# aleju/cat-generator

Measured on AMD Instinct MI355X. Metric: images/sec per G+D step, G32up-c 32x32 RGB bs=128 per GPU, higher is better.
Workload: dtype f32

## Files before the change

cat-generator_amd/csrc/common.h:

```cpp
#pragma once
#include <hip/hip_runtime.h>
#include <algorithm>
#include <stdint.h>
#include <stdio.h>
#include <string.h>
#include "../../include/catgan.h"

namespace cg {

char* err_buf();
int fail(const char* fmt, ...);

inline hipStream_t S(void* s) { return reinterpret_cast<hipStream_t>(s); }

#define CG_HIP(call)                                                              \
    do {                                                                          \
        hipError_t e__ = (call);                                                  \
        if (e__ != hipSuccess)                                                    \
            return cg::fail("%s:%d %s -> %s", __FILE__, __LINE__, #call,          \
                            hipGetErrorString(e__));                              \
    } while (0)

#define CG_LAUNCH_CHECK()                                                         \
    do {                                                                          \
        hipError_t e__ = hipGetLastError();                                       \
        if (e__ != hipSuccess)                                                    \
            return cg::fail("%s:%d kernel launch -> %s", __FILE__, __LINE__,      \
                            hipGetErrorString(e__));                              \
    } while (0)

#define CG_REQUIRE(cond, ...)                                                     \
    do {                                                                          \
        if (!(cond)) return cg::fail(__VA_ARGS__);                                \
    } while (0)

constexpr int kNumCU = 256;

#ifndef CG_TIMING_PROBE
#define CG_TIMING_PROBE 0
#endif
#define CG_PROBE_HALF(fam, T) (((CG_TIMING_PROBE) & (fam)) ? ((T) + 1) / 2 : (T))
constexpr int kEwWgsPerCU = 4, kColReduceWgsPerCU = 1;

enum Opt {
    OPT_SKINNY, OPT_GEMM_BK32, OPT_WINO_BK, OPT_NN_TILE, OPT_TN_TILE, OPT_NN_SPLITS, OPT_TN_SPLITS,
    OPT_XCD_SWIZZLE, OPT_NN_GLDS, OPT_TN_GLDS, OPT_WINO_GLDS, OPT_PAD_SKIP, OPT_WINO3, OPT_COUNT
};
long opt(Opt o);

static inline int cdiv(long a, long b) { return (int)((a + b - 1) / b); }

constexpr size_t kColScratchBytes = 8u << 20;
void* col_scratch(hipStream_t stream);
hipStream_t queue_stream(hipStream_t ref, int cls, int slot);
int queue_class(hipStream_t ref, hipStream_t s);
void wgrad_discard_all();

bool skinny_mfma_ok(int Cin, int Cout, int H, int W);
int skinny_mfma_forward(hipStream_t st, const float* x, const float* w, const float* bias, float* y, int N, int H, int W, int Cin, int Cout);
int skinny_mfma_wgrad(hipStream_t st, const float* x, const float* dy, float* part, float* bias_part, int N, int H, int W, int Cin, int Cout,
                      int max_blocks);

bool head_wgrad_ok(int N, int T, int C, int Co);
int head_wgrad(hipStream_t st, const float* x, const float* dy, float* gw, float* gb, int N, int T, int C, int Co, float scale);
bool wino3_geom_ok(int ngroups, int N, int H, int W, int Cin, int Cout, int kH, int kW, int padH, int padW, int ups);
int wino3_note_pack(hipStream_t st, int n, const float* const* w, float* const* wf, float* const* wb, const int* Cout, const int* Cin,
                    const int* kH, const int* kW, const int* wb_map);
int wino3_forward(hipStream_t st, int ngroups, const float* const* x, const float* const* wpk, const float* const* bias, float* const* y,
                  int N, int H, int W);

static inline int ew_grid(long n, int per_block = 256) {
    long b = (n + per_block - 1) / per_block;
    if (b < 1) b = 1;
    const long cap = (long)kNumCU * kEwWgsPerCU;
    if (b > cap) b = cap;
    return (int)b;
}

__device__ __forceinline__ float u01(uint64_t seed, uint64_t ctr) {
    uint64_t z = seed + (ctr + 1) * 0x9E3779B97F4A7C15ull;
    z = (z ^ (z >> 30)) * 0xBF58476D1CE4E5B9ull;
    z = (z ^ (z >> 27)) * 0x94D049BB133111EBull;
    z = z ^ (z >> 31);
    return (float)(z >> 40) * (1.0f / 16777216.0f);
}
__device__ __forceinline__ float wave_sum(float v) {
#pragma unroll
    for (int off = 32; off > 0; off >>= 1) v += __shfl_down(v, off, 64);
    return v;
// ... 112 lines not shown
```

cat-generator_amd/csrc/gemm.hip:

```cpp
#include "common.h"
#include <stdlib.h>
#include <algorithm>
#include <mutex>
#include <type_traits>
#include <unordered_map>
#include <vector>

namespace {

typedef float f32x16 __attribute__((ext_vector_type(16)));
typedef unsigned int u32x4 __attribute__((ext_vector_type(4)));

constexpr int BK = 16;
constexpr unsigned OOB = 0x80000000u;
#ifdef CG_TRACE
__device__ unsigned long long* g_trace;
#define CG_STAMP(slot)                                                                                                  \
    do {                                                                                                                \
        if (threadIdx.x == 0 && g_trace) {                                                                              \
            const long wg = blockIdx.x + (long)gridDim.x * (blockIdx.y + (long)gridDim.y * blockIdx.z);                  \
            g_trace[wg * 8 + (slot)] = wall_clock64();                                                                  \
            if ((slot) == 0) {                                                                                          \
                g_trace[wg * 8 + 4] = __builtin_amdgcn_s_getreg((31 << 11) | 4);                       \
                g_trace[wg * 8 + 5] = __builtin_amdgcn_s_getreg((31 << 11) | 20);                     \
// ... 1320 lines not shown
#pragma unroll
            for (int r = 0; r < 16; ++r) {
                const int soff = (i * 32 + (r & 3) + 8 * (r >> 2)) * c4;
#pragma unroll
                for (int j = 0; j < NI; ++j)
                    __builtin_amdgcn_raw_buffer_store_b32(__float_as_uint(acc[i][j][r]), rp, (int)(vo + j * 128), soff, 0);
            }
        return;
    }
#pragma unroll
    for (int j = 0; j < NI; ++j) {
        const int n = n0 + wn0 + j * 32 + l31;
        if (n >= g.Cout) continue;
#pragma unroll
        for (int i = 0; i < MI; ++i) {
#pragma unroll
            for (int r = 0; r < 16; ++r) {
                const int m = m0 + wm0 + i * 32 + (r & 3) + 8 * (r >> 2) + 4 * h;
                if (m < g.Ktot) pout[(long)m * g.Cout + n] = acc[i][j][r];
            }
        }
    }
}

__device__ __host__ __forceinline__ int phase_map(int a, int d, int pad) { return ((a + d - pad) >> 1) - ((a - pad) >> 1); }

template <bool UPS>
__global__ __launch_bounds__(256) void wgrad_reduce_kernel(const float* part, float* gw, int Cin, int Cout, int k, int KK,
                                                           int pad, int kp, int S, float scale, int CI_T, long sstride) {
    extern __shared__ float sh[];
    const int ci0 = blockIdx.x * CI_T, co0 = blockIdx.y * 32;
    const long plane = (long)(UPS ? kp * kp : KK) * Cin * Cout;
    const int n1 = KK * CI_T * 32;
    if (UPS && k == 3 && kp == 2 && pad == 1 && co0 + 32 <= Cout && ci0 + CI_T <= Cin && (CI_T & 31) == 0 && (Cout & 3) == 0 && ((uintptr_t)part & 15) == 0 &&
        (sstride & 3) == 0) {
        const int c4 = threadIdx.x & 7;
        for (int ci_l = threadIdx.x >> 3; ci_l < CI_T; ci_l += 32) {
            float4 acc[9];
#pragma unroll
            for (int t = 0; t < 9; ++t) acc[t] = make_float4(0.f, 0.f, 0.f, 0.f);
            const float* base = part + (long)(ci0 + ci_l) * Cout + co0 + 4 * c4;
            for (int sp = 0; sp < S; ++sp) {
                float4 v[4][4];
#pragma unroll
                for (int p = 0; p < 4; ++p)
#pragma unroll
                    for (int tp = 0; tp < 4; ++tp) v[p][tp] = ld4(base + (long)sp * sstride + (long)p * plane + (long)tp * Cin * Cout);
#pragma unroll
                for (int t = 0; t < 9; ++t) {
                    const int dy = t / 3, dx = t - 3 * (t / 3);
#pragma unroll
                    for (int p = 0; p < 4; ++p) {
                        const float4 q = v[p][phase_map(p >> 1, dy, 1) * 2 + phase_map(p & 1, dx, 1)];
                        acc[t].x += q.x; acc[t].y += q.y; acc[t].z += q.z; acc[t].w += q.w;
                    }
                }
            }
#pragma unroll
            for (int t = 0; t < 9; ++t) {
                float* d = sh + (ci_l * KK + t) * 33 + 4 * c4;
                d[0] = acc[t].x; d[1] = acc[t].y; d[2] = acc[t].z; d[3] = acc[t].w;
            }
        }
    } else
    for (int idx = threadIdx.x; idx < n1; idx += 256) {
        const int co_l = idx & 31;
        const int r = idx >> 5;
        const int ci_l = r % CI_T, tap = r / CI_T;
        const int ci = ci0 + ci_l, co = co0 + co_l;
        float s = 0.f;
        if (ci < Cin && co < Cout) {
            if (UPS) {
                const int dy = tap / k, dx = tap - dy * k;
                for (int sp = 0; sp < S; ++sp)
#pragma unroll
                    for (int p = 0; p < 4; ++p) {
                        const int tp = phase_map(p >> 1, dy, pad) * kp + phase_map(p & 1, dx, pad);
                        s += part[(long)sp * sstride + (long)p * plane + ((long)tp * Cin + ci) * Cout + co];
                    }
            } else {
                const long o = ((long)tap * Cin + ci) * Cout + co;
                for (int sp = 0; sp < S; ++sp) s += part[(long)sp * sstride + o];
            }
        }
        sh[(ci_l * KK + tap) * 33 + co_l] = s;
    }
    __syncthreads();
    const int run = CI_T * KK;
    for (int idx = threadIdx.x; idx < n1; idx += 256) {
        const int j = idx % run, co_l = idx / run;
        const int ci_l = j / KK, tap = j - ci_l * KK;
        const int ci = ci0 + ci_l, co = co0 + co_l;
        if (ci < Cin && co < Cout) {
            float* dst = gw + ((long)co * Cin + ci) * KK + tap;
            *dst += scale * sh[j * 33 + co_l];
        }
    }
}

struct RedPtrs { float* gw0; float* gw1; float* gw2; float* gw3; float* gb0; float* gb1; float* gb2; float* gb3;
                 long gws; };

template <bool UPS>
__device__ __forceinline__ void wgrad_reduce_small_body(float (*sh)[33], int bx, int group, const float* part, const float* bias_part,
                                                        const RedPtrs& rp, int Cin, int Cout, int k, int KK, int pad, int kp, int S,
                                                        int P, float scale, long sstride, long gstride, long bsstride, int wblocks) {
    const int ol = threadIdx.x & 31, ln = threadIdx.x >> 5;
    float s = 0.f;
    if (bx < wblocks) {
        const long total = (long)KK * Cin * Cout;
        const long plane = (long)(UPS ? kp * kp : KK) * Cin * Cout;
        const long i = bx * 32L + ol;
        const float* pg = part + (long)group * gstride;
        int co = 0, ci = 0, tap = 0;
        if (i < total) {
            co = (int)(i % Cout);
            const long r = i / Cout;
            ci = (int)(r % Cin);
            tap = (int)(r / Cin);
            if (UPS) {
                const int dy = tap / k, dx = tap - dy * k;
                for (int sp = ln; sp < S; sp += 8)
#pragma unroll
                    for (int p = 0; p < 4; ++p) {
                        const int tp = phase_map(p >> 1, dy, pad) * kp + phase_map(p & 1, dx, pad);
                        s += pg[(long)sp * sstride + (long)p * plane + ((long)tp * Cin + ci) * Cout + co];
                    }
            } else {
#pragma unroll 4
// ... 970 lines not shown
size_t cg_conv2d_wgrad_workspace_bytes(int N, int Hp, int Wp, int Cin, int Cout, int kH, int kW, int padH, int padW,
                                       int ups) {
    return cg_conv2d_wgrad_workspace_bytes_grouped(1, N, Hp, Wp, Cin, Cout, kH, kW, padH, padW, ups);
}

namespace {
std::mutex g_red_mu;
std::unordered_map<hipStream_t, std::vector<RedJob>> g_red_queue;

long red_cap() { return 0x7fffffffL; }

int small_reduce(hipStream_t st, bool defer, const RedJob& job, int ngroups) {
    if (defer) {
        std::lock_guard<std::mutex> lk(g_red_mu);
        g_red_queue[st].push_back(job);
        g_red_queue[st].back().block0 = ngroups;
        return 0;
    }
    const int nblocks = job.wblocks + job.bblocks;
    const long cap = std::max<long>(1, red_cap() / std::max(1, ngroups));
    dim3 sgrid((unsigned)std::min<long>(nblocks, cap), ngroups);
    if (job.ups)
        hipLaunchKernelGGL(wgrad_reduce_small_kernel<true>, sgrid, dim3(256), 0, st, job.part, job.bias_part, job.rp, job.Cin, job.Cout,
                           job.k, job.KK, job.pad, job.kp, job.S, job.P, job.scale, job.sstride, job.gstride, job.bsstride, job.wblocks, nblocks, 0);
    else
        hipLaunchKernelGGL(wgrad_reduce_small_kernel<false>, sgrid, dim3(256), 0, st, job.part, job.bias_part, job.rp, job.Cin, job.Cout,
                           job.k, job.KK, job.pad, job.kp, job.S, job.P, job.scale, job.sstride, job.gstride, job.bsstride, job.wblocks, nblocks, job.v4);
    CG_LAUNCH_CHECK();
    return 0;
}

int wgrad_impl(void* stream, int ngroups, const float* const* x, const float* const* dy, float* const* gw, float* const* gb, int N,
               int Hp, int Wp, int Cin, int Cout, int kH, int kW, int padH, int padW, int ups, float scale, void* ws, size_t ws_bytes,
               bool defer, long xgs = 0, long dgs = 0, long gws = 0, bool gemm_only = false);
}

int cg_conv2d_wgrad_grouped(void* stream, int ngroups, const float* const* x, const float* const* dy, float* const* gw,
                            float* const* gb, int N, int Hp, int Wp, int Cin, int Cout, int kH, int kW, int padH, int padW,
                            int ups, float scale, void* ws, size_t ws_bytes) {
    return wgrad_impl(stream, ngroups, x, dy, gw, gb, N, Hp, Wp, Cin, Cout, kH, kW, padH, padW, ups, scale, ws, ws_bytes, false);
}

int cg_conv2d_wgrad_grouped_deferred(void* stream, int ngroups, const float* const* x, const float* const* dy, float* const* gw,
                                     float* const* gb, int N, int Hp, int Wp, int Cin, int Cout, int kH, int kW, int padH, int padW,
                                     int ups, float scale, void* ws, size_t ws_bytes) {
    return wgrad_impl(stream, ngroups, x, dy, gw, gb, N, Hp, Wp, Cin, Cout, kH, kW, padH, padW, ups, scale, ws, ws_bytes, true);
}

int cg_conv2d_wgrad_strided(void* stream, int ngroups, const float* x, long x_stride, const float* dy, long dy_stride, float* gw,
                            long gw_stride, int N, int Hp, int Wp, int Cin, int Cout, int kH, int kW, int padH, int padW, int ups,
                            float scale, void* ws, size_t ws_bytes) {
    CG_REQUIRE(x && dy && gw && x_stride > 0 && dy_stride > 0 && gw_stride > 0, "cg_conv2d_wgrad_strided: bad arguments");
    CG_REQUIRE(ngroups >= 1 && ngroups <= kMaxStridedGroups, "cg_conv2d_wgrad_strided: 1..%d groups per launch", kMaxStridedGroups);
    return wgrad_impl(stream, ngroups, &x, &dy, &gw, nullptr, N, Hp, Wp, Cin, Cout, kH, kW, padH, padW, ups, scale, ws, ws_bytes, false,
                      x_stride, dy_stride, gw_stride);
}

int cg_conv2d_wgrad_gemm(void* stream, const float* x, const float* dy, int N, int Hp, int Wp, int Cin, int Cout, int kH, int kW, int padH,
                         int padW, int ups, void* ws, size_t ws_bytes) {
    CG_REQUIRE(x && dy && ws, "cg_conv2d_wgrad_gemm: null pointer");
    CG_REQUIRE(!skinny_ok(1, Cin, Cout, kH, kW, padH, padW, ups), "cg_conv2d_wgrad_gemm: this geometry runs the skinny kernel, not the GEMM");
    float* gw = (float*)ws;
    return wgrad_impl(stream, 1, &x, &dy, &gw, nullptr, N, Hp, Wp, Cin, Cout, kH, kW, padH, padW, ups, 1.f, ws, ws_bytes, false, 0, 0, 0, true);
}

int cg_conv2d_wgrad_pending(void* stream, int* njobs) {
    CG_REQUIRE(njobs, "cg_conv2d_wgrad_pending: null pointer");
    std::lock_guard<std::mutex> lk(g_red_mu);
    auto it = g_red_queue.find(cg::S(stream));
    *njobs = it == g_red_queue.end() ? 0 : (int)it->second.size();
    return 0;
}

int cg_conv2d_wgrad_flush(void* stream) {
    hipStream_t st = cg::S(stream);
    std::vector<RedJob> jobs;
    {
        std::lock_guard<std::mutex> lk(g_red_mu);
        auto it = g_red_queue.find(st);
        if (it == g_red_queue.end() || it->second.empty()) return 0;
        jobs.swap(it->second);
    }
    for (size_t j0 = 0; j0 < jobs.size(); j0 += kRedJobs) {
        RedJobTable t;
        memset(&t, 0, sizeof(t));
        t.n = (int)std::min<size_t>(kRedJobs, jobs.size() - j0);
        int blocks = 0;
        for (int q = 0; q < t.n; ++q) {
            t.j[q] = jobs[j0 + q];
            const int ngroups = t.j[q].block0;
            t.j[q].block0 = blocks;
            blocks += ngroups * (t.j[q].wblocks + t.j[q].bblocks);
        }
        const int wgs = (int)std::min<long>(blocks, red_cap());
        hipLaunchKernelGGL(wgrad_reduce_batch_kernel, dim3(wgs), dim3(256), 0, st, t, blocks);
        CG_LAUNCH_CHECK();
    }
    return 0;
}

namespace {
int wgrad_impl(void* stream, int ngroups, const float* const* x, const float* const* dy, float* const* gw, float* const* gb, int N,
               int Hp, int Wp, int Cin, int Cout, int kH, int kW, int padH, int padW, int ups, float scale, void* ws, size_t ws_bytes,
               bool defer, long xgs, long dgs, long gws_, bool gemm_only) {
    CG_REQUIRE(x && dy && gw, "cg_conv2d_wgrad: null pointer");
    const bool strided = xgs != 0;
    CG_REQUIRE(ngroups >= 1 && ngroups <= (strided ? kMaxStridedGroups : MAXG), "cg_conv2d_wgrad: 1..%d groups per launch", strided ? kMaxStridedGroups : MAXG);
    CG_REQUIRE(!strided || (!gb && !defer), "cg_conv2d_wgrad: strided groups carry no bias gradient and are not deferred");
    TNArgs a;
    memset(&a, 0, sizeof(a));
    if (conv_geom(a.g, N, Hp, Wp, Cin, Cout, kH, kW, padH, padW, ups)) return 1;
    const Geom& g = a.g;
    if (!strided && skinny_ok(ngroups, Cin, Cout, kH, kW, padH, padW, ups) && x[0] && dy[0] && gw[0] && (uintptr_t)x[0] % 16 == 0 && ws &&
        ws_bytes >= skinny_wgrad_ws_bytes(Cin, Cout) && (long)N * Hp * Wp < 0x7fffffffL) {
        hipStream_t st = cg::S(stream);
        const long npix = (long)N * Hp * Wp;
        const long ppb = (npix + kSkinnyWgradBlocks - 1) / kSkinnyWgradBlocks;
        int blocks = (int)((npix + ppb - 1) / ppb);
        float* part = (float*)ws;
        float* bpart = part + (size_t)kSkinnyWgradBlocks * 9 * Cin * Cout;
        float* gb0 = gb ? gb[0] : nullptr;
        if (cg::opt(cg::OPT_SKINNY) == 1 && cg::skinny_mfma_ok(Cin, Cout, Hp, Wp)) {
            blocks = cg::skinny_mfma_wgrad(st, x[0], dy[0], part, gb0 ? bpart : nullptr, N, Hp, Wp, Cin, Cout, kSkinnyWgradBlocks / 2);
            if (blocks < 0) return 1;
        }
        else if (Cout == 3) skinny_wgrad_launch<3>(st, x[0], dy[0], part, gb0 ? bpart : nullptr, N, Hp, Wp, Cin, blocks, ppb);
        else skinny_wgrad_launch<1>(st, x[0], dy[0], part, gb0 ? bpart : nullptr, N, Hp, Wp, Cin, blocks, ppb);
        CG_LAUNCH_CHECK();
        RedJob job;
        memset(&job, 0, sizeof(job));
        job.part = part; job.bias_part = bpart;
        job.rp.gw0 = gw[0]; job.rp.gb0 = gb0;
        job.Cin = Cin; job.Cout = Cout; job.k = 3; job.KK = 9; job.pad = 1; job.S = blocks; job.P = 1; job.scale = scale;
        job.sstride = 9L * Cin * Cout; job.gstride = 0; job.bsstride = Cout;
        job.wblocks = cg::cdiv(9L * Cin * Cout, 32); job.bblocks = gb0 ? cg::cdiv(Cout, 32) : 0;
        return small_reduce(st, defer, job, 1);
    }
// ... 10 lines not shown
    for (int i = 0; i < (strided ? 1 : ngroups); ++i) {
        CG_REQUIRE(x[i] && dy[i] && gw[i], "cg_conv2d_wgrad: null pointer (group %d)", i);
        xs[i] = x[i]; ds[i] = dy[i];
        veca = veca && ((uintptr_t)x[i] % 16 == 0);
        vecb = vecb && ((uintptr_t)dy[i] % 16 == 0);
        any_gb = any_gb || (gb && gb[i]);
    }
    if (strided) { veca = veca && xgs % 4 == 0; vecb = vecb && dgs % 4 == 0; }
    if (p.pm && !(veca && vecb)) p = plan_tn(g, ngroups, false);
    a.xgs = xgs; a.dgs = dgs;
    a.x0 = xs[0]; a.x1 = xs[1]; a.x2 = xs[2]; a.x3 = xs[3];
    a.d0 = ds[0]; a.d1 = ds[1]; a.d2 = ds[2]; a.d3 = ds[3];
    a.ngroups = ngroups; a.part = (float*)ws; a.pchunk = p.pchunk;
    a.xcd_swizzle = (int)cg::opt(cg::OPT_XCD_SWIZZLE);
    const int ZP = ngroups * g.nphase;
    const long wplane = (long)g.Ktot * g.Cout;
    a.bias_part = any_gb ? (float*)ws + (size_t)p.splits * ZP * wplane : nullptr;
    hipStream_t st = cg::S(stream);
    dim3 grid(cg::cdiv(g.Ktot, p.tc.bm) * cg::cdiv(g.Cout, p.tc.bn), p.splits, ZP);
    if (p.pm && veca && vecb) a.pm_n = g.M / (g.Hg * g.Wg);
    if (a.pm_n || tng_ok(g, p.pchunk, veca, vecb)) {
        if (p.tc.bm == 128 && p.tc.bn == 128) launch_tng<128, 128, 2, 2>(a, grid, st);
        else if (p.tc.bm == 64 && p.tc.bn == 128) launch_tng<64, 128, 2, 2>(a, grid, st);
        else if (p.tc.bm == 128 && p.tc.bn == 64) launch_tng<128, 64, 2, 2>(a, grid, st);
        else if (p.tc.bm == 64 && p.tc.bn == 64) launch_tng<64, 64, 2, 2>(a, grid, st);
        else launch_tng<128, 32, 4, 1>(a, grid, st);
    }
    else if (p.tc.bm == 128 && p.tc.bn == 128) launch_tn<128, 128, 2, 2>(a, grid, st, veca, vecb);
    else if (p.tc.bm == 64 && p.tc.bn == 128) launch_tn<64, 128, 2, 2>(a, grid, st, veca, vecb);
    else if (p.tc.bm == 128 && p.tc.bn == 64) launch_tn<128, 64, 2, 2>(a, grid, st, veca, vecb);
    else if (p.tc.bm == 64 && p.tc.bn == 64) launch_tn<64, 64, 2, 2>(a, grid, st, veca, vecb);
    else launch_tn<128, 32, 4, 1>(a, grid, st, veca, vecb);
    CG_LAUNCH_CHECK();
    if (gemm_only) return 0;
    const int KK = kH * kW;
    int ci_t = KK == 1 ? 64 : 8;
    while (ci_t > 1 && (size_t)KK * ci_t * 33 * sizeof(float) > 60000) ci_t >>= 1;
    const size_t shb = (size_t)KK * ci_t * 33 * sizeof(float);
    dim3 rgrid(cg::cdiv(Cin, ci_t), cg::cdiv(Cout, 32));
    const long relems = (long)KK * Cin * Cout;
    const long sstride = (long)ZP * wplane;
    const int kp = ups ? phase_kp(kH, padH) : 0;
    if (strided && KK == 1 && !ups && !any_gb && Cin % 32 == 0 && Cout % 32 == 0 && g.nphase == 1) {
        hipLaunchKernelGGL(wgrad_reduce_t_kernel, dim3(Cin / 32, Cout / 32, ngroups), dim3(256), 0, st, (const float*)ws, gw[0], gws_, Cin, Cout,
                           p.splits, sstride, (long)g.nphase * wplane, scale);
        CG_LAUNCH_CHECK();
        return 0;
    }
    if ((long)rgrid.x * rgrid.y < cg::kNumCU) {
        RedJob job;
        memset(&job, 0, sizeof(job));
        float* gws[MAXG] = {nullptr, nullptr, nullptr, nullptr};
        float* gbs[MAXG] = {nullptr, nullptr, nullptr, nullptr};
        for (int gi = 0; gi < (strided ? 1 : ngroups); ++gi) { gws[gi] = gw[gi]; gbs[gi] = gb ? gb[gi] : nullptr; }
        job.rp.gws = strided ? gws_ : 0;
        job.rp.gw0 = gws[0]; job.rp.gw1 = gws[1]; job.rp.gw2 = gws[2]; job.rp.gw3 = gws[3];
        job.rp.gb0 = gbs[0]; job.rp.gb1 = gbs[1]; job.rp.gb2 = gbs[2]; job.rp.gb3 = gbs[3];
        job.part = (const float*)ws; job.bias_part = a.bias_part;
        job.Cin = Cin; job.Cout = Cout; job.k = kH; job.KK = KK; job.pad = padH; job.kp = ups ? kp : 0; job.S = p.splits; job.P = g.nphase;
        job.ups = ups ? 1 : 0; job.scale = scale;
        job.sstride = sstride; job.gstride = (long)g.nphase * wplane; job.bsstride = (long)ZP * Cout;
        job.wblocks = cg::cdiv(relems, 32); job.bblocks = any_gb ? cg::cdiv(Cout, 32) : 0;
        if (defer && KK == 1 && !ups && Cin % 32 == 0 && Cout % 32 == 0 && g.nphase == 1) {
            job.tr = 1; job.wblocks = (Cin / 32) * (Cout / 32);
        } else if (!ups && Cout % 4 == 0 && (uintptr_t)ws % 16 == 0 && sstride % 4 == 0 && job.gstride % 4 == 0) {
            job.v4 = 1; job.wblocks = cg::cdiv(relems, 128);
        }
        return small_reduce(st, defer, job, ngroups);
    }
    for (int gi = 0; gi < ngroups; ++gi) {
        const float* pg = (const float*)ws + (long)gi * g.nphase * wplane;
        float* gwi = strided ? gw[0] + (long)gi * gws_ : gw[gi];
        if (ups)
            hipLaunchKernelGGL(wgrad_reduce_kernel<true>, rgrid, dim3(256), shb, st, pg, gwi, Cin, Cout, kH, KK, padH, kp,
                               p.splits, scale, ci_t, sstride);
        else
            hipLaunchKernelGGL(wgrad_reduce_kernel<false>, rgrid, dim3(256), shb, st, pg, gwi, Cin, Cout, kH, KK, padH,
                               0, p.splits, scale, ci_t, sstride);
        CG_LAUNCH_CHECK();
        if (gb && gb[gi]) {
            hipLaunchKernelGGL(bias_part_reduce_kernel, dim3(cg::cdiv(Cout, 32)), dim3(256), 0, st,
                               (const float*)a.bias_part + (long)gi * g.nphase * Cout, gb[gi], p.splits, g.nphase,
                               (long)ZP * Cout, Cout, scale);
            CG_LAUNCH_CHECK();
        }
    }
    return 0;
}

}

int cg_conv2d_wgrad(void* stream, const float* x, const float* dy, float* gw, float* gb, int N, int Hp, int Wp, int Cin,
                    int Cout, int kH, int kW, int padH, int padW, int ups, float scale, void* ws, size_t ws_bytes) {
    CG_REQUIRE(x && dy && gw, "cg_conv2d_wgrad: null pointer");
    return cg_conv2d_wgrad_grouped(stream, 1, &x, &dy, &gw, &gb, N, Hp, Wp, Cin, Cout, kH, kW, padH, padW, ups, scale, ws,
                                   ws_bytes);
}

static int pack_ci_tile(int Cin, int KK) {
    int t = 1;
    while (t * 2 * KK <= 448 && t < Cin) t *= 2;
    return t;
}

int cg_pack_conv_weight(void* stream, const float* w, float* wf, float* wb, int Cout, int Cin, int kH, int kW) {
// ... 80 lines not shown
```

cat-generator_amd/csrc/winograd.hip:

```cpp
#include "common.h"
#include <algorithm>
#include <type_traits>
#include <stdlib.h>

namespace {

typedef float f32x16 __attribute__((ext_vector_type(16)));

__device__ __forceinline__ float4 ld4(const float* p) { return *reinterpret_cast<const float4*>(p); }
__device__ __forceinline__ float wf4c(const float4& v, int i) { return i == 0 ? v.x : (i == 1 ? v.y : (i == 2 ? v.z : v.w)); }
__device__ __forceinline__ float4 f4add(float4 a, float4 b) { return make_float4(a.x + b.x, a.y + b.y, a.z + b.z, a.w + b.w); }
__device__ __forceinline__ float4 f4sub(float4 a, float4 b) { return make_float4(a.x - b.x, a.y - b.y, a.z - b.z, a.w - b.w); }

template <int MODE>
__global__ __launch_bounds__(256) void wino_input_transform_kernel(const float* __restrict__ src, float* __restrict__ V,
                                                                   int N, int Hl, int Wl, int C, int Cs) {
    const int cq_n = C >> 2;
    const int tH = Hl >> 1, tW = Wl >> 1;
    const long T = (long)N * tH * tW;
    const long total = T * cq_n;
    for (long idx = blockIdx.x * 256L + threadIdx.x; idx < total; idx += gridDim.x * 256L) {
        const int cq = (int)(idx % cq_n);
        const long tile = idx / cq_n;
        const int tj = (int)(tile % tW);
// ... 595 lines not shown
        const int cq = (int)((blockIdx.x * 256L + threadIdx.x) % cq_n);
        if (cq_n >= 256) *reinterpret_cast<float4*>(bpart + (long)blockIdx.x * C + cq * 4) = bacc;
        else if ((int)threadIdx.x < cq_n) {
            float4 t = shb[threadIdx.x];
            for (int j = threadIdx.x + cq_n; j < 256; j += cq_n) t = f4add(t, shb[j]);
            *reinterpret_cast<float4*>(bpart + (long)blockIdx.x * C + cq * 4) = t;
        }
    }
}

__global__ __launch_bounds__(256) void wino_bias_finish_kernel(const float* __restrict__ bpart, int nblocks, int Cout, float* __restrict__ gb,
                                                               float scale) {
    __shared__ double sh[8][33];
    const int cl = threadIdx.x & 31, rl = threadIdx.x >> 5;
    const int co = blockIdx.x * 32 + cl;
    double a = 0.0;
    if (co < Cout)
        for (int b = rl; b < nblocks; b += 8) {
            const float* row = bpart + (long)b * 4 * Cout + co;
            a += ((double)row[0] + (double)row[Cout]) + ((double)row[2 * Cout] + (double)row[3 * Cout]);
        }
    sh[rl][cl] = a;
    __syncthreads();
    if (rl == 0 && co < Cout) {
        double t = 0.0;
#pragma unroll
        for (int r = 0; r < 8; ++r) t += sh[r][cl];
        gb[co] += scale * (float)t;
    }
}

__device__ __host__ __forceinline__ int wino_phase_map(int a, int d) { return ((a + d - 2) >> 1) - ((a - 2) >> 1); }

__global__ __launch_bounds__(256) void wino_wgrad_finish_kernel(const float* __restrict__ dUt, float* __restrict__ gw, int Cout,
                                                                int Cin, float scale) {
    const long total = (long)Cout * Cin;
    const long xs = 4L * Cout * Cin;
    for (long idx = blockIdx.x * 256L + threadIdx.x; idx < total; idx += gridDim.x * 256L) {
        const int ci = (int)(idx % Cin);
        const int co = (int)(idx / Cin);
        float acc[25];
#pragma unroll
        for (int t = 0; t < 25; ++t) acc[t] = 0.f;
#pragma unroll
        for (int p = 0; p < 4; ++p) {
            float u[4][4];
#pragma unroll
            for (int xi = 0; xi < 16; ++xi) u[xi >> 2][xi & 3] = dUt[xi * xs + ((long)p * Cout + co) * Cin + ci];
            float t[3][4];
#pragma unroll
            for (int c = 0; c < 4; ++c) {
                t[0][c] = u[0][c] + 0.5f * (u[1][c] + u[2][c]);
                t[1][c] = 0.5f * (u[1][c] - u[2][c]);
                t[2][c] = 0.5f * (u[1][c] + u[2][c]) + u[3][c];
            }
            float g[3][3];
#pragma unroll
            for (int r = 0; r < 3; ++r) {
                g[r][0] = t[r][0] + 0.5f * (t[r][1] + t[r][2]);
                g[r][1] = 0.5f * (t[r][1] - t[r][2]);
                g[r][2] = 0.5f * (t[r][1] + t[r][2]) + t[r][3];
            }
#pragma unroll
            for (int dy = 0; dy < 5; ++dy)
#pragma unroll
                for (int dx = 0; dx < 5; ++dx) acc[dy * 5 + dx] += g[wino_phase_map(p >> 1, dy)][wino_phase_map(p & 1, dx)];
        }
        float* dst = gw + idx * 25;
#pragma unroll
        for (int t = 0; t < 25; ++t) dst[t] += scale * acc[t];
    }
}


__device__ __host__ __forceinline__ int wino22_phase_map(int a, int d) { return ((a + d - 1) >> 1) - ((a - 1) >> 1); }


static bool wino_dims_ok(int N, int Hp, int Wp, int Cin, int Cout) {
    return N > 0 && Hp > 0 && Wp > 0 && (Hp & 1) == 0 && (Wp & 1) == 0 && Cin > 0 && Cout > 0 && Cin % 128 == 0 &&
           Cout % 128 == 0  && (long)N * Hp * Wp * std::max(Cin, 4 * Cout) * 4L < (1L << 40);
}

}

extern "C" {

size_t cg_conv2d_ups2_wino_supported(int N, int Hp, int Wp, int Cin, int Cout, int k, int pad) {
    return k == 5 && pad == 2 && wino_dims_ok(N, Hp, Wp, Cin, Cout) ? 1 : 0;
}
size_t cg_conv2d_ups2_wino_v_floats(int N, int Hp, int Wp, int C) {
    return (size_t)16 * ((size_t)N * (Hp / 2) * (Wp / 2)) * C;
}
size_t cg_conv2d_ups2_wino_u_floats(int Cin, int Cout) { return (size_t)4 * 16 * Cin * Cout; }

int cg_conv2d_ups2_wino_pack(void* stream, const float* wf_ph, const float* wb_ph, float* u_fwd, float* u_bwd, int Cout,
                             int Cin) {
    CG_REQUIRE((wf_ph && u_fwd) || (wb_ph && u_bwd), "cg_conv2d_ups2_wino_pack: null pointer");
    CG_REQUIRE(Cin % 4 == 0 && Cout % 4 == 0, "cg_conv2d_ups2_wino_pack: channel counts must be multiples of 4");
    if (wf_ph && u_fwd) {
        const long total = 4L * Cin * (Cout / 4);
        hipLaunchKernelGGL(wino_filter_transform_kernel<false>, dim3(cg::ew_grid(total)), dim3(256), 0, cg::S(stream), wf_ph,
                           u_fwd, Cin, Cout);
        CG_LAUNCH_CHECK();
// ... 175 lines not shown
    const bool glds = cg::opt(cg::OPT_WINO_GLDS) != 0 && T * 4L * Cout * 4L < 0x7fffffffL &&
                      16L * 4L * Cout * Cin * 4L < 0x7fffffffL;
    if (!glds || !wino_dims_ok(N, Hp, Wp, Cin, Cout)) return 1;
    const long wgs = (long)cg::cdiv((int)T, 64) * (Cin / 128);
    int sl = force == 1 || force == 2 || force == 4 ? force : (wgs >= cg::kNumCU ? 1 : (wgs * 2 >= cg::kNumCU ? 2 : 4));
    while (sl > 1 && (4 * Cout / sl) % 64 != 0) sl >>= 1;
    return sl;
}
size_t cg_conv2d_ups2_wino_dgrad_part_floats(int N, int Hp, int Wp, int Cin, int Cout) {
    const int sl = wino_dgrad_slices(N, Hp, Wp, Cin, Cout);
    return sl > 1 ? (size_t)sl * N * Hp * Wp * Cin : 0;
}
int cg_conv2d_ups2_wino_dgrad_split(void* stream, const float* dy, const float* u_bwd, float* dx_lo, float* v_dy, float* part, int N, int Hp,
                                    int Wp, int Cin, int Cout) {
    const int sl = wino_dgrad_slices(N, Hp, Wp, Cin, Cout);
    if (sl <= 1 || !part) return cg_conv2d_ups2_wino_dgrad(stream, dy, u_bwd, dx_lo, v_dy, N, Hp, Wp, Cin, Cout);
    CG_REQUIRE(dy && u_bwd && dx_lo && v_dy, "cg_conv2d_ups2_wino_dgrad_split: null pointer");
    const int T = N * (Hp / 2) * (Wp / 2);
    hipLaunchKernelGGL(wino_input_transform_kernel<1>, dim3(cg::ew_grid((long)T * Cout)), dim3(256), 0, cg::S(stream), dy, v_dy, N, Hp, Wp, 4 * Cout, Cout);
    CG_LAUNCH_CHECK();
    if (wino_gemm_launch(stream, v_dy, u_bwd, nullptr, part, N, Hp, Wp, Cin, Cout, 1, nullptr, 16, sl)) return 1;
    const long n = (long)T * 4 * Cin;
    if (sl == 4) hipLaunchKernelGGL(wino22_sum_kernel<4>, dim3(cg::ew_grid(n / 4)), dim3(256), 0, cg::S(stream), part, dx_lo, n / 4, n);
    else hipLaunchKernelGGL(wino22_sum_kernel<2>, dim3(cg::ew_grid(n / 4)), dim3(256), 0, cg::S(stream), part, dx_lo, n / 4, n);
    CG_LAUNCH_CHECK();
    return 0;
}

static size_t wino_align(size_t b) { return (b + 255) / 256 * 256; }

size_t cg_conv2d_ups2_wino_wgrad_workspace_bytes(int N, int Hp, int Wp, int Cin, int Cout) {
    if (!wino_dims_ok(N, Hp, Wp, Cin, Cout)) return 0;
    const size_t T = (size_t)N * (Hp / 2) * (Wp / 2);
    return wino_align(16 * T * 4 * Cout * sizeof(float)) + wino_align((size_t)16 * 4 * Cout * Cin * sizeof(float)) +
           wino_align(std::max(sizeof(double) * Cout, (size_t)cg::kNumCU * 8 * 4 * Cout * sizeof(float))) +

           cg_conv2d_wgrad_workspace_bytes_strided(16, (int)T, 1, 1, Cin, 4 * Cout, 1, 1, 0, 0, 0);
}

int cg_conv2d_ups2_wino_wgrad(void* stream, const float* v, const float* dy, float* gw_canonical, float* gb, int N, int Hp,
                              int Wp, int Cin, int Cout, float scale, void* ws, size_t ws_bytes) {
    CG_REQUIRE(v && dy && gw_canonical, "cg_conv2d_ups2_wino_wgrad: null pointer");
    CG_REQUIRE(wino_dims_ok(N, Hp, Wp, Cin, Cout), "cg_conv2d_ups2_wino_wgrad: unsupported dimensions");
    const size_t need = cg_conv2d_ups2_wino_wgrad_workspace_bytes(N, Hp, Wp, Cin, Cout);
    CG_REQUIRE(ws && ws_bytes >= need && (uintptr_t)ws % 16 == 0, "cg_conv2d_ups2_wino_wgrad: workspace too small (%zu < %zu)",
               ws_bytes, need);
    hipStream_t st = cg::S(stream);
    const int T = N * (Hp / 2) * (Wp / 2);
    const int C4 = 4 * Cout;
    char* base = (char*)ws;
    float* mdy = (float*)base;                    base += wino_align((size_t)16 * T * C4 * sizeof(float));
    float* dut = (float*)base;                    base += wino_align((size_t)16 * C4 * Cin * sizeof(float));
    const size_t bws_bytes = wino_align(std::max(sizeof(double) * Cout, (size_t)cg::kNumCU * 8 * 4 * Cout * sizeof(float)));
    void* bws = base;                             base += bws_bytes;
    void* tws = base;
    const size_t tws_bytes = ws_bytes - (size_t)(base - (char*)ws);
    const bool fuse = false;
    const int tgrid = (int)cg::ew_grid((long)T * Cout);
    hipLaunchKernelGGL(wino_dy_transform_kernel, dim3(tgrid), dim3(256), 0, st, dy, mdy, N, Hp, Wp, Cout, fuse ? (float*)bws : nullptr);
    CG_LAUNCH_CHECK();
    CG_HIP(hipMemsetAsync(dut, 0, (size_t)16 * C4 * Cin * sizeof(float), st));
    const int groups_per_launch = 16;
    for (int q = 0; q < 16; q += groups_per_launch) {
        if (cg_conv2d_wgrad_strided(stream, groups_per_launch, v + q * (long)T * Cin, (long)T * Cin, mdy + q * (long)T * C4, (long)T * C4,
                                    dut + q * (long)C4 * Cin, (long)C4 * Cin, T, 1, 1, Cin, C4, 1, 1, 0, 0, 0, 1.f, tws, tws_bytes)) return 1;
    }
    hipLaunchKernelGGL(wino_wgrad_finish_kernel, dim3(cg::ew_grid((long)Cout * Cin)), dim3(256), 0, st, dut, gw_canonical, Cout,
                       Cin, scale);
    CG_LAUNCH_CHECK();
    if (fuse) {
        hipLaunchKernelGGL(wino_bias_finish_kernel, dim3(cg::cdiv(Cout, 32)), dim3(256), 0, st, (const float*)bws, tgrid, Cout, gb, scale);
        CG_LAUNCH_CHECK();
        return 0;
    }
    if (gb) return cg_bias_grad(stream, dy, gb, (long)N * 4 * Hp * Wp, Cout, scale, bws, wino_align(sizeof(double) * Cout));
    return 0;
}



}
```

Baseline: 22970.

## Fuse split-K reduction into Winograd wgrad finish and add dedicated ups3 reduce kernel

Result: faster. 23280 (median of 6 runs) (+1.3%).

```diff
diff --git a/cat-generator_amd/csrc/common.h b/cat-generator_amd/csrc/common.h
--- a/cat-generator_amd/csrc/common.h
+++ b/cat-generator_amd/csrc/common.h
@@ -55,6 +55,8 @@
 hipStream_t queue_stream(hipStream_t ref, int cls, int slot);
 int queue_class(hipStream_t ref, hipStream_t s);
 void wgrad_discard_all();
+int wgrad_strided_partials(void* stream, int ngroups, const float* x, long x_stride, const float* dy, long dy_stride, int N, int Cin,
+                           int Cout, void* ws, size_t ws_bytes, int* splits);
 
 bool skinny_mfma_ok(int Cin, int Cout, int H, int W);
 int skinny_mfma_forward(hipStream_t st, const float* x, const float* w, const float* bias, float* y, int N, int H, int W, int Cin, int Cout);
diff --git a/cat-generator_amd/csrc/gemm.hip b/cat-generator_amd/csrc/gemm.hip
--- a/cat-generator_amd/csrc/gemm.hip
+++ b/cat-generator_amd/csrc/gemm.hip
@@ -1376,37 +1376,6 @@
     const int ci0 = blockIdx.x * CI_T, co0 = blockIdx.y * 32;
     const long plane = (long)(UPS ? kp * kp : KK) * Cin * Cout;
     const int n1 = KK * CI_T * 32;
-    if (UPS && k == 3 && kp == 2 && pad == 1 && co0 + 32 <= Cout && ci0 + CI_T <= Cin && (CI_T & 31) == 0 && (Cout & 3) == 0 && ((uintptr_t)part & 15) == 0 &&
-        (sstride & 3) == 0) {
-        const int c4 = threadIdx.x & 7;
-        for (int ci_l = threadIdx.x >> 3; ci_l < CI_T; ci_l += 32) {
-            float4 acc[9];
-#pragma unroll
-            for (int t = 0; t < 9; ++t) acc[t] = make_float4(0.f, 0.f, 0.f, 0.f);
-            const float* base = part + (long)(ci0 + ci_l) * Cout + co0 + 4 * c4;
-            for (int sp = 0; sp < S; ++sp) {
-                float4 v[4][4];
-#pragma unroll
-                for (int p = 0; p < 4; ++p)
-#pragma unroll
-                    for (int tp = 0; tp < 4; ++tp) v[p][tp] = ld4(base + (long)sp * sstride + (long)p * plane + (long)tp * Cin * Cout);
-#pragma unroll
-                for (int t = 0; t < 9; ++t) {
-                    const int dy = t / 3, dx = t - 3 * (t / 3);
-#pragma unroll
-                    for (int p = 0; p < 4; ++p) {
-                        const float4 q = v[p][phase_map(p >> 1, dy, 1) * 2 + phase_map(p & 1, dx, 1)];
-                        acc[t].x += q.x; acc[t].y += q.y; acc[t].z += q.z; acc[t].w += q.w;
-                    }
-                }
-            }
-#pragma unroll
-            for (int t = 0; t < 9; ++t) {
-                float* d = sh + (ci_l * KK + t) * 33 + 4 * c4;
-                d[0] = acc[t].x; d[1] = acc[t].y; d[2] = acc[t].z; d[3] = acc[t].w;
-            }
-        }
-    } else
     for (int idx = threadIdx.x; idx < n1; idx += 256) {
         const int co_l = idx & 31;
         const int r = idx >> 5;
@@ -1439,6 +1408,85 @@
             float* dst = gw + ((long)co * Cin + ci) * KK + tap;
             *dst += scale * sh[j * 33 + co_l];
         }
+    }
+}
+
+constexpr int kUps3CiT = 16;
+__device__ __forceinline__ void ups3_load(float4 (&v)[16], __amdgpu_buffer_rsrc_t r, unsigned voff, int soff, int plane4, int tstride4) {
+#pragma unroll
+    for (int p = 0; p < 4; ++p)
+#pragma unroll
+        for (int tp = 0; tp < 4; ++tp) v[p * 4 + tp] = bufld4(r, voff, soff + p * plane4 + tp * tstride4);
+}
+__device__ __forceinline__ void ups3_add(float4 (&acc)[9], const float4 (&v)[16]) {
+#pragma unroll
+    for (int t = 0; t < 9; ++t) {
+        const int dy = t / 3, dx = t - 3 * (t / 3);
+#pragma unroll
+        for (int p = 0; p < 4; ++p) {
+            const float4 q = v[p * 4 + phase_map(p >> 1, dy, 1) * 2 + phase_map(p & 1, dx, 1)];
+            acc[t].x += q.x; acc[t].y += q.y; acc[t].z += q.z; acc[t].w += q.w;
+        }
+    }
+}
+__global__ __launch_bounds__(128) void wgrad_reduce_ups3_kernel(const float* __restrict__ part, const float* __restrict__ bias_part,
+                                                                float* __restrict__ gw, float* __restrict__ gb, int Cin, int Cout, int S,
+                                                                int P, float scale, long sstride, long bsstride, int wblocks) {
+    __shared__ float sh[kUps3CiT * 9][33];
+    const int b = (int)blockIdx.x;
+    if (b >= wblocks) {
+        const int cl = threadIdx.x & 15, ln = threadIdx.x >> 4;
+        const int c = (b - wblocks) * 16 + cl;
+        float s = 0.f;
+        if (c < Cout)
+            for (int i = ln; i < S * P; i += 8) s += bias_part[(long)(i / P) * bsstride + (long)(i % P) * Cout + c];
+        sh[ln][cl] = s;
+        __syncthreads();
+        if (ln == 0 && c < Cout) {
+            float t = 0.f;
+#pragma unroll
+            for (int r = 0; r < 8; ++r) t += sh[r][cl];
+            gb[c] += scale * t;
+        }
+        return;
+    }
+    const int nco = Cout / 32;
+    const int ci0 = (b / nco) * kUps3CiT, co0 = (b - (b / nco) * nco) * 32;
+    const int tstride4 = Cin * Cout * 4, plane4 = 4 * tstride4, sstride4 = (int)(sstride * 4);
+    const int c4 = threadIdx.x & 7, ci_l = threadIdx.x >> 3;
+    const __amdgpu_buffer_rsrc_t rs = __builtin_amdgcn_make_buffer_rsrc((void*)(part + (long)ci0 * Cout + co0), 0, 0x7fffffff, 0x00020000);
+    const unsigned voff = (unsigned)(ci_l * Cout + 4 * c4) * 4u;
+    float4 acc[9];
+#pragma unroll
+    for (int t = 0; t < 9; ++t) acc[t] = make_float4(0.f, 0.f, 0.f, 0.f);
+    float4 va[16], vb[16];
+    ups3_load(va, rs, voff, 0, plane4, tstride4);
+#pragma unroll 1
+    for (int sp = 0; sp + 2 < S; sp += 2) {
+        ups3_load(vb, rs, voff, (sp + 1) * sstride4, plane4, tstride4);
+        __builtin_amdgcn_sched_barrier(0);
+        ups3_add(acc, va);
+        __builtin_amdgcn_sched_barrier(0);
+        ups3_load(va, rs, voff, (sp + 2) * sstride4, plane4, tstride4);
+        __builtin_amdgcn_sched_barrier(0);
+        ups3_add(acc, vb);
+        __builtin_amdgcn_sched_barrier(0);
+    }
+    ups3_load(vb, rs, voff, (S - 1) * sstride4, plane4, tstride4);
+    __builtin_amdgcn_sched_barrier(0);
+    ups3_add(acc, va);
+    ups3_add(acc, vb);
+#pragma unroll
+    for (int t = 0; t < 9; ++t) {
+        float* d = &sh[ci_l * 9 + t][4 * c4];
+        d[0] = acc[t].x; d[1] = acc[t].y; d[2] = acc[t].z; d[3] = acc[t].w;
+    }
+    __syncthreads();
+    constexpr int run = kUps3CiT * 9;
+    for (int idx = threadIdx.x; idx < run * 32; idx += 128) {
+        const int j = idx % run, co_l = idx / run;
+        float* dst = gw + ((long)(co0 + co_l) * Cin + ci0) * 9 + j;
+        *dst += scale * sh[j][co_l];
     }
 }
 
@@ -2475,7 +2523,7 @@
 
 int wgrad_impl(void* stream, int ngroups, const float* const* x, const float* const* dy, float* const* gw, float* const* gb, int N,
                int Hp, int Wp, int Cin, int Cout, int kH, int kW, int padH, int padW, int ups, float scale, void* ws, size_t ws_bytes,
-               bool defer, long xgs = 0, long dgs = 0, long gws = 0, bool gemm_only = false);
+               bool defer, long xgs = 0, long dgs = 0, long gws = 0, bool gemm_only = false, int* splits_out = nullptr);
 }
 
 int cg_conv2d_wgrad_grouped(void* stream, int ngroups, const float* const* x, const float* const* dy, float* const* gw,
@@ -2506,6 +2554,19 @@
     float* gw = (float*)ws;
     return wgrad_impl(stream, 1, &x, &dy, &gw, nullptr, N, Hp, Wp, Cin, Cout, kH, kW, padH, padW, ups, 1.f, ws, ws_bytes, false, 0, 0, 0, true);
 }
+
+}
+namespace cg {
+int wgrad_strided_partials(void* stream, int ngroups, const float* x, long x_stride, const float* dy, long dy_stride, int N, int Cin,
+                           int Cout, void* ws, size_t ws_bytes, int* splits) {
+    CG_REQUIRE(x && dy && ws && splits && x_stride > 0 && dy_stride > 0, "wgrad_strided_partials: bad arguments");
+    CG_REQUIRE(ngroups >= 1 && ngroups <= kMaxStridedGroups, "wgrad_strided_partials: 1..%d groups per launch", kMaxStridedGroups);
+    float* gw = (float*)ws;
+    return wgrad_impl(stream, ngroups, &x, &dy, &gw, nullptr, N, 1, 1, Cin, Cout, 1, 1, 0, 0, 0, 1.f, ws, ws_bytes, false, x_stride,
+                      dy_stride, 1, true, splits);
+}
+}
+extern "C" {
 
 int cg_conv2d_wgrad_pending(void* stream, int* njobs) {
     CG_REQUIRE(njobs, "cg_conv2d_wgrad_pending: null pointer");
@@ -2545,7 +2606,7 @@
 namespace {
 int wgrad_impl(void* stream, int ngroups, const float* const* x, const float* const* dy, float* const* gw, float* const* gb, int N,
                int Hp, int Wp, int Cin, int Cout, int kH, int kW, int padH, int padW, int ups, float scale, void* ws, size_t ws_bytes,
-               bool defer, long xgs, long dgs, long gws_, bool gemm_only) {
+               bool defer, long xgs, long dgs, long gws_, bool gemm_only, int* splits_out) {
     CG_REQUIRE(x && dy && gw, "cg_conv2d_wgrad: null pointer");
     const bool strided = xgs != 0;
     CG_REQUIRE(ngroups >= 1 && ngroups <= (strided ? kMaxStridedGroups : MAXG), "cg_conv2d_wgrad: 1..%d groups per launch", strided ? kMaxStridedGroups : MAXG);
@@ -2622,6 +2683,7 @@
     else if (p.tc.bm == 64 && p.tc.bn == 64) launch_tn<64, 64, 2, 2>(a, grid, st, veca, vecb);
     else launch_tn<128, 32, 4, 1>(a, grid, st, veca, vecb);
     CG_LAUNCH_CHECK();
+    if (splits_out) *splits_out = p.splits;
     if (gemm_only) return 0;
     const int KK = kH * kW;
     int ci_t = KK == 1 ? 64 : 8;
@@ -2658,9 +2720,21 @@
         }
         return small_reduce(st, defer, job, ngroups);
     }
+    const bool ups3 = ups && kH == 3 && padH == 1 && kp == 2 && g.nphase == 4 && Cin % kUps3CiT == 0 && Cout % 32 == 0 &&
+                      p.splits % 2 == 0 && (uintptr_t)ws % 16 == 0 && (long)p.splits * sstride * 4 < 0x7fffffffL;
     for (int gi = 0; gi < ngroups; ++gi) {
         const float* pg = (const float*)ws + (long)gi * g.nphase * wplane;
         float* gwi = strided ? gw[0] + (long)gi * gws_ : gw[gi];
+        if (ups3) {
+            float* gbi = gb ? gb[gi] : nullptr;
+            const int wblocks = (Cin / kUps3CiT) * (Cout / 32);
+            const int blocks = wblocks + (gbi ? cg::cdiv(Cout, 16) : 0);
+            hipLaunchKernelGGL(wgrad_reduce_ups3_kernel, dim3(blocks), dim3(128), 0, st, pg,
+                               gbi ? (const float*)a.bias_part + (long)gi * g.nphase * Cout : nullptr, gwi, gbi, Cin, Cout, p.splits,
+                               g.nphase, scale, sstride, (long)ZP * Cout, wblocks);
+            CG_LAUNCH_CHECK();
+            continue;
+        }
         if (ups)
             hipLaunchKernelGGL(wgrad_reduce_kernel<true>, rgrid, dim3(256), shb, st, pg, gwi, Cin, Cout, kH, KK, padH, kp,
                                p.splits, scale, ci_t, sstride);
diff --git a/cat-generator_amd/csrc/winograd.hip b/cat-generator_amd/csrc/winograd.hip
--- a/cat-generator_amd/csrc/winograd.hip
+++ b/cat-generator_amd/csrc/winograd.hip
@@ -651,43 +651,101 @@
 
 __device__ __host__ __forceinline__ int wino_phase_map(int a, int d) { return ((a + d - 2) >> 1) - ((a - 2) >> 1); }
 
-__global__ __launch_bounds__(256) void wino_wgrad_finish_kernel(const float* __restrict__ dUt, float* __restrict__ gw, int Cout,
-                                                                int Cin, float scale) {
-    const long total = (long)Cout * Cin;
-    const long xs = 4L * Cout * Cin;
-    for (long idx = blockIdx.x * 256L + threadIdx.x; idx < total; idx += gridDim.x * 256L) {
-        const int ci = (int)(idx % Cin);
-        const int co = (int)(idx / Cin);
-        float acc[25];
+typedef unsigned wu32x4 __attribute__((ext_vector_type(4)));
+typedef float wf32x4 __attribute__((ext_vector_type(4)));
+__device__ __forceinline__ float4 wbufld4(__amdgpu_buffer_rsrc_t r, unsigned voff, int soff) {
+    const wf32x4 f = __builtin_bit_cast(wf32x4, __builtin_amdgcn_raw_buffer_load_b128(r, voff, soff, 0));
+    return make_float4(f.x, f.y, f.z, f.w);
+}
+constexpr int kWinoFinCiT = 4;
+__device__ __forceinline__ void wino_wgrad_phase(const float (&u)[4][4], float (&acc)[25], int p) {
+    float t[3][4];
+#pragma unroll
+    for (int c = 0; c < 4; ++c) {
+        t[0][c] = u[0][c] + 0.5f * (u[1][c] + u[2][c]);
+        t[1][c] = 0.5f * (u[1][c] - u[2][c]);
+        t[2][c] = 0.5f * (u[1][c] + u[2][c]) + u[3][c];
+    }
+    float g[3][3];
+#pragma unroll
+    for (int r = 0; r < 3; ++r) {
+        g[r][0] = t[r][0] + 0.5f * (t[r][1] + t[r][2]);
+        g[r][1] = 0.5f * (t[r][1] - t[r][2]);
+        g[r][2] = 0.5f * (t[r][1] + t[r][2]) + t[r][3];
+    }
+#pragma unroll
+    for (int dy = 0; dy < 5; ++dy)
+#pragma unroll
+        for (int dx = 0; dx < 5; ++dx) acc[dy * 5 + dx] += g[wino_phase_map(p >> 1, dy)][wino_phase_map(p & 1, dx)];
+}
+
+__global__ __launch_bounds__(256) void wino_wgrad_finish_kernel(const float* __restrict__ part, float* __restrict__ gw, int Cout, int Cin,
+                                                                int S, float scale) {
+    __shared__ __attribute__((aligned(16))) float sh[4 * 16 * kWinoFinCiT * 32];
+    const int nco = Cout / 32;
+    const int ci0 = ((int)blockIdx.x / nco) * kWinoFinCiT, co0 = ((int)blockIdx.x - ((int)blockIdx.x / nco) * nco) * 32;
+    const int C4 = 4 * Cout;
+    const long gstride = (long)Cin * C4, sstride = 16 * gstride;
+    {
+        const int c4 = threadIdx.x & 7, r8 = threadIdx.x >> 3;
+        const __amdgpu_buffer_rsrc_t rs = __builtin_amdgcn_make_buffer_rsrc((void*)(part + (long)ci0 * C4 + co0), 0, 0x7fffffff, 0x00020000);
+        unsigned vo[8];
+#pragma unroll
+        for (int j = 0; j < 8; ++j) {
+            const int row = r8 + 32 * j, ci_l = row & 3, xi = (row >> 2) & 15, p = row >> 6;
+            vo[j] = (unsigned)(xi * (int)gstride + ci_l * C4 + p * Cout + 4 * c4) * 4u;
+        }
+        const int ss4 = (int)(sstride * 4);
+        float4 s[8];
+#pragma unroll
+        for (int j = 0; j < 8; ++j) s[j] = make_float4(0.f, 0.f, 0.f, 0.f);
+        int sp = 0;
+        for (; sp + 2 <= S; sp += 2) {
+            float4 v0[8], v1[8];
+#pragma unroll
+            for (int j = 0; j < 8; ++j) v0[j] = wbufld4(rs, vo[j], sp * ss4);
+#pragma unroll
+            for (int j = 0; j < 8; ++j) v1[j] = wbufld4(rs, vo[j], (sp + 1) * ss4);
+#pragma unroll
+            for (int j = 0; j < 8; ++j) {
+                s[j].x += v0[j].x; s[j].y += v0[j].y; s[j].z += v0[j].z; s[j].w += v0[j].w;
+                s[j].x += v1[j].x; s[j].y += v1[j].y; s[j].z += v1[j].z; s[j].w += v1[j].w;
+            }
+        }
+        if (sp < S)
+#pragma unroll
+            for (int j = 0; j < 8; ++j) {
+                const float4 v = wbufld4(rs, vo[j], sp * ss4);
+                s[j].x += v.x; s[j].y += v.y; s[j].z += v.z; s[j].w += v.w;
+            }
+#pragma unroll
+        for (int j = 0; j < 8; ++j) *reinterpret_cast<float4*>(&sh[(r8 + 32 * j) * 32 + 4 * c4]) = s[j];
+    }
+    __syncthreads();
+    float acc[25];
+    const int co_l = threadIdx.x & 31, ci_l = threadIdx.x >> 5;
+    if (threadIdx.x < 32 * kWinoFinCiT) {
 #pragma unroll
         for (int t = 0; t < 25; ++t) acc[t] = 0.f;
 #pragma unroll
         for (int p = 0; p < 4; ++p) {
             float u[4][4];
 #pragma unroll
-            for (int xi = 0; xi < 16; ++xi) u[xi >> 2][xi & 3] = dUt[xi * xs + ((long)p * Cout + co) * Cin + ci];
-            float t[3][4];
-#pragma unroll
-            for (int c = 0; c < 4; ++c) {
-                t[0][c] = u[0][c] + 0.5f * (u[1][c] + u[2][c]);
-                t[1][c] = 0.5f * (u[1][c] - u[2][c]);
-                t[2][c] = 0.5f * (u[1][c] + u[2][c]) + u[3][c];
-            }
-            float g[3][3];
-#pragma unroll
-            for (int r = 0; r < 3; ++r) {
-                g[r][0] = t[r][0] + 0.5f * (t[r][1] + t[r][2]);
-                g[r][1] = 0.5f * (t[r][1] - t[r][2]);
-                g[r][2] = 0.5f * (t[r][1] + t[r][2]) + t[r][3];
-            }
-#pragma unroll
-            for (int dy = 0; dy < 5; ++dy)
-#pragma unroll
-                for (int dx = 0; dx < 5; ++dx) acc[dy * 5 + dx] += g[wino_phase_map(p >> 1, dy)][wino_phase_map(p & 1, dx)];
-        }
-        float* dst = gw + idx * 25;
-#pragma unroll
-        for (int t = 0; t < 25; ++t) dst[t] += scale * acc[t];
+            for (int xi = 0; xi < 16; ++xi) u[xi >> 2][xi & 3] = sh[((p * 16 + xi) * 4 + ci_l) * 32 + co_l];
+            wino_wgrad_phase(u, acc, p);
+        }
+    }
+    __syncthreads();
+    constexpr int run = kWinoFinCiT * 25;
+    if (threadIdx.x < 32 * kWinoFinCiT) {
+#pragma unroll
+        for (int t = 0; t < 25; ++t) sh[co_l * (run + 1) + ci_l * 25 + t] = acc[t];
+    }
+    __syncthreads();
+    for (int idx = threadIdx.x; idx < 32 * run; idx += 256) {
+        const int c = idx / run, j = idx - c * run;
+        float* dst = gw + ((long)(co0 + c) * Cin + ci0) * 25 + j;
+        *dst += scale * sh[c * (run + 1) + j];
     }
 }
 
@@ -929,7 +987,7 @@
 size_t cg_conv2d_ups2_wino_wgrad_workspace_bytes(int N, int Hp, int Wp, int Cin, int Cout) {
     if (!wino_dims_ok(N, Hp, Wp, Cin, Cout)) return 0;
     const size_t T = (size_t)N * (Hp / 2) * (Wp / 2);
-    return wino_align(16 * T * 4 * Cout * sizeof(float)) + wino_align((size_t)16 * 4 * Cout * Cin * sizeof(float)) +
+    return wino_align(16 * T * 4 * Cout * sizeof(float)) +
            wino_align(std::max(sizeof(double) * Cout, (size_t)cg::kNumCU * 8 * 4 * Cout * sizeof(float))) +
 
            cg_conv2d_wgrad_workspace_bytes_strided(16, (int)T, 1, 1, Cin, 4 * Cout, 1, 1, 0, 0, 0);
@@ -947,7 +1005,6 @@
     const int C4 = 4 * Cout;
     char* base = (char*)ws;
     float* mdy = (float*)base;                    base += wino_align((size_t)16 * T * C4 * sizeof(float));
-    float* dut = (float*)base;                    base += wino_align((size_t)16 * C4 * Cin * sizeof(float));
     const size_t bws_bytes = wino_align(std::max(sizeof(double) * Cout, (size_t)cg::kNumCU * 8 * 4 * Cout * sizeof(float)));
     void* bws = base;                             base += bws_bytes;
     void* tws = base;
@@ -956,14 +1013,11 @@
     const int tgrid = (int)cg::ew_grid((long)T * Cout);
     hipLaunchKernelGGL(wino_dy_transform_kernel, dim3(tgrid), dim3(256), 0, st, dy, mdy, N, Hp, Wp, Cout, fuse ? (float*)bws : nullptr);
     CG_LAUNCH_CHECK();
-    CG_HIP(hipMemsetAsync(dut, 0, (size_t)16 * C4 * Cin * sizeof(float), st));
-    const int groups_per_launch = 16;
-    for (int q = 0; q < 16; q += groups_per_launch) {
-        if (cg_conv2d_wgrad_strided(stream, groups_per_launch, v + q * (long)T * Cin, (long)T * Cin, mdy + q * (long)T * C4, (long)T * C4,
-                                    dut + q * (long)C4 * Cin, (long)C4 * Cin, T, 1, 1, Cin, C4, 1, 1, 0, 0, 0, 1.f, tws, tws_bytes)) return 1;
-    }
-    hipLaunchKernelGGL(wino_wgrad_finish_kernel, dim3(cg::ew_grid((long)Cout * Cin)), dim3(256), 0, st, dut, gw_canonical, Cout,
-                       Cin, scale);
+    int splits = 0;
+    if (cg::wgrad_strided_partials(stream, 16, v, (long)T * Cin, mdy, (long)T * C4, T, Cin, C4, tws, tws_bytes, &splits)) return 1;
+    CG_REQUIRE((long)splits * 16 * Cin * C4 * 4 < 0x7fffffffL, "cg_conv2d_ups2_wino_wgrad: %d split planes span 2 GB or more", splits);
+    hipLaunchKernelGGL(wino_wgrad_finish_kernel, dim3((Cin / kWinoFinCiT) * (Cout / 32)), dim3(256), 0, st, (const float*)tws, gw_canonical,
+                       Cout, Cin, splits, scale);
     CG_LAUNCH_CHECK();
     if (fuse) {
         hipLaunchKernelGGL(wino_bias_finish_kernel, dim3(cg::cdiv(Cout, 32)), dim3(256), 0, st, (const float*)bws, tgrid, Cout, gb, scale);
```
